# DeepRec-AI/DeepRec

Measured on AMD Instinct MI355X. Metric: samples/sec (whole node) DLRM Criteo-TB-shaped synthetic, higher is better.
Workload: dtype bf16; 1 GPU; model=dlrm, global_batch=8192, seq_len=1, parallelism=single, hip_graph=True, optimizer=adamasync, embedding_dim=16, num_tables=26

## Files before the change

### deeprec_amd/ops/hip/dense_kernels.hip

```cpp

#include "hip_common.h"

#include <algorithm>

namespace py = pybind11;

namespace {

using bf16 = __hip_bfloat16;
using bf16x8 = __attribute__((ext_vector_type(8))) short;
using f32x4 = __attribute__((ext_vector_type(4))) float;

__device__ __forceinline__ short act_grad_u16(short g, short o, int act) {
  const float ov = bf2f_u16(o);
  if (act == 1) return ov > 0.0f ? g : (short)0;
  return f2bf_u16(bf2f_u16(g) * ov * (1.0f - ov));
}

__device__ __forceinline__ bf16x8 load_frag_row(const short* __restrict__ src,
                                                int r, int k0, int rows,
                                                int cols) {
  bf16x8 out;
  if (r < rows && k0 + 7 < cols) {
    const short* p = src + (int64_t)r * cols + k0;
    out = *reinterpret_cast<const bf16x8*>(p);
  } else {
#pragma unroll
    for (int i = 0; i < 8; ++i) {
      short v = 0;
      if (r < rows && k0 + i < cols) v = src[(int64_t)r * cols + k0 + i];
      out[i] = v;
    }
  }
  return out;
}

__device__ __forceinline__ bf16x8 load_frag_col(const short* __restrict__ src,
                                                int c, int k0, int rows,
                                                int cols) {
  bf16x8 out;
#pragma unroll
  for (int i = 0; i < 8; ++i) {
    short v = 0;
    int r = k0 + i;
    if (r < rows && c < cols) v = src[(int64_t)r * cols + c];
    out[i] = v;
  }
  return out;
}

using bf16x4 = __attribute__((ext_vector_type(4))) short;
constexpr int TRT_COLS = 64;

__device__ __forceinline__ int trt_off(int row, int col) {
  const int sw = ((row >> 1) & 1) | ((row >> 2) & 2);
  return row * TRT_COLS + ((((col >> 4) ^ sw) << 4) | (col & 15));
}

__device__ __forceinline__ int trt_lane_off(int lane, int cb) {
  return trt_off(8 * (lane >> 4) + ((lane >> 2) & 3), cb + 4 * (lane & 3));
}

__device__ __forceinline__ bf16x4 lds_read_tr16(const short* p) {
  return __builtin_amdgcn_ds_read_tr16_b64_v4i16(
      (__attribute__((address_space(3))) bf16x4*)p);
}

__device__ __forceinline__ bf16x8 trt_frag(const short* p) {
  const bf16x4 lo = lds_read_tr16(p);
  const bf16x4 hi = lds_read_tr16(p + 4 * TRT_COLS);
  return __builtin_shufflevector(lo, hi, 0, 1, 2, 3, 4, 5, 6, 7);
}

constexpr int TRT_STAGE_THREADS = 256;
static_assert(TRT_STAGE_THREADS / 8 == 32, "a slab is 32 rows of 8 segments");
struct TrtStager {
  int row, col, off;
  __device__ __forceinline__ explicit TrtStager(int tid)
      : row(tid >> 3), col((tid & 7) * 8), off(trt_off(row, col)) {}
  __device__ __forceinline__ bf16x8 load(const short* __restrict__ src,
                                         int row0, int slab, int col0,
                                         int rows, int cols) const {
    return load_frag_row(src, row0 + slab * 32 + row, col0 + col, rows, cols);
  }
  __device__ __forceinline__ void store(short* tile, int slab,
                                        bf16x8 v) const {
    *reinterpret_cast<bf16x8*>(&tile[slab * 32 * TRT_COLS + off]) = v;
  }
};


__device__ __forceinline__ short fwd_act_u16(float acc, float bv, int act) {
  float v = acc + bv;
  if (act == 1 && v < 0.0f) v = 0.0f;
  else if (act == 2) v = 1.0f / (1.0f + __expf(-v));
  return f2bf_u16(v);
}

__device__ __forceinline__ void dx_store_tile(
    const f32x4 (&acc)[4], int lane, int m0, int c0, int kt, int M, int K,
    short* __restrict__ dX, const short* __restrict__ prev_out,
    int prev_act) {
#pragma unroll
  for (int t = 0; t < 4; ++t) {
    if (t >= kt) break;
    const int ck = c0 + t * 16 + (lane & 15);
    if (ck >= K) continue;
#pragma unroll
    for (int i = 0; i < 4; ++i) {
      int cm = m0 + (lane >> 4) * 4 + i;
      if (cm >= M) continue;
      short v = f2bf_u16(acc[t][i]);
      if (prev_out)
        v = act_grad_u16(v, prev_out[(int64_t)cm * K + ck], prev_act);
      dX[(int64_t)cm * K + ck] = v;
    }
  }
}

template <int NT>
__device__ __forceinline__ void dw_flush(const f32x4 (&acc)[NT], int lane,
                                         int n0, int k0, int N, int K,
                                         float* __restrict__ dW) {
#pragma unroll
  for (int t = 0; t < NT; ++t) {
    const int ck = k0 + t * 16 + (lane & 15);
    if (ck >= K) continue;
#pragma unroll
    for (int i = 0; i < 4; ++i) {
      int cn = n0 + (lane >> 4) * 4 + i;
      if (cn >= N) continue;
      atomicAdd(&dW[(int64_t)cn * K + ck], acc[t][i]);
    }
  }
}

__device__ __forceinline__ float dbias_add_frag(float bsum, bf16x8 gfrag) {
#pragma unroll
  for (int i = 0; i < 8; ++i) bsum += bf2f_u16(gfrag[i]);
  return bsum;
}

__device__ __forceinline__ void dbias_reduce_add(float bsum, int lane, int n0,
                                                 int N,
                                                 float* __restrict__ dbias) {
  float v = bsum;
  for (int off = 16; off < 64; off += 16)
    v += __shfl(bsum, (lane & 15) + off);
  const int cn = n0 + (lane & 15);
  if (lane < 16 && cn < N) atomicAdd(&dbias[cn], v);
}

template <int MT>
__global__ void k_linear_fwd_t(const short* __restrict__ A,
                               const short* __restrict__ W,
                               const float* __restrict__ bias, int M, int N,
                               int K, int act, short* __restrict__ C) {
  const int lane = threadIdx.x & 63;
  const int wave = threadIdx.x >> 6;
  const int ntiles64 = (N + 63) / 64;
  const int m0 = (blockIdx.x / ntiles64) * 64 * MT + wave * 16 * MT;
  const int n0 = (blockIdx.x % ntiles64) * 64;
  if (m0 >= M) return;
  const int col_b = n0 + (lane & 15);
  const int kgrp = (lane >> 4) * 8;
  f32x4 acc[MT][4] = {};
  const int nt = min(4, (N - n0 + 15) / 16);
  for (int k0 = 0; k0 < K; k0 += 32) {
    bf16x8 a[MT];
#pragma unroll
    for (int r = 0; r < MT; ++r)
      a[r] = load_frag_row(A, m0 + r * 16 + (lane & 15), k0 + kgrp, M, K);
#pragma unroll
    for (int t = 0; t < 4; ++t) {
      if (t >= nt) break;
      bf16x8 b = load_frag_row(W, col_b + t * 16, k0 + kgrp, N, K);
#pragma unroll
      for (int r = 0; r < MT; ++r)
        acc[r][t] = __builtin_amdgcn_mfma_f32_16x16x32_bf16(a[r], b,
                                                            acc[r][t], 0, 0,
                                                            0);
    }
  }
  __shared__ short cstage[4][16][72];
  const bool full_tile =
      (MT == 1) && (n0 + 64 <= N) && (m0 + 16 <= M) && ((N & 7) == 0);
  if (full_tile) {
#pragma unroll
    for (int t = 0; t < 4; ++t) {
      const int cn = t * 16 + (lane & 15);
      const float bv = bias ? bias[n0 + cn] : 0.0f;
#pragma unroll
      for (int i = 0; i < 4; ++i) {
        cstage[wave][(lane >> 4) * 4 + i][cn] =
            fwd_act_u16(acc[0][t][i], bv, act);
      }
    }
    __builtin_amdgcn_s_waitcnt(0);
#pragma unroll
    for (int half = 0; half < 2; ++half) {
      const int row = half * 8 + (lane >> 3);
      const int c8 = (lane & 7) * 8;
      bf16x8 vreg;
#pragma unroll
      for (int j = 0; j < 8; ++j) vreg[j] = cstage[wave][row][c8 + j];
      *reinterpret_cast<bf16x8*>(
          C + (int64_t)(m0 + row) * N + n0 + c8) = vreg;
    }
    return;
  }
#pragma unroll
  for (int r = 0; r < MT; ++r) {
#pragma unroll
    for (int t = 0; t < 4; ++t) {
      if (t >= nt) break;
      const int cn = n0 + t * 16 + (lane & 15);
      if (cn >= N) continue;
      const float bv = bias ? bias[cn] : 0.0f;
#pragma unroll
      for (int i = 0; i < 4; ++i) {
        int cm = m0 + r * 16 + (lane >> 4) * 4 + i;
        if (cm >= M) continue;
        C[(int64_t)cm * N + cn] = fwd_act_u16(acc[r][t][i], bv, act);
      }
    }
  }
}

__global__ void k_linear_dx(const short* __restrict__ G,
                            const short* __restrict__ W, int M, int N, int K,
                            short* __restrict__ dX,
                            const short* __restrict__ prev_out,
                            int prev_act) {
  const int lane = threadIdx.x & 63;
  const int wave = threadIdx.x >> 6;
  const int ktiles64 = (K + 63) / 64;
  const int m0 = (blockIdx.x / ktiles64) * 64 + wave * 16;
  const int c0 = (blockIdx.x % ktiles64) * 64;
  if (m0 >= M) return;
  const int row_g = m0 + (lane & 15);
  const int col_w = c0 + (lane & 15);
  const int kgrp = (lane >> 4) * 8;
  f32x4 acc[4] = {{0.f, 0.f, 0.f, 0.f}, {0.f, 0.f, 0.f, 0.f},
                  {0.f, 0.f, 0.f, 0.f}, {0.f, 0.f, 0.f, 0.f}};
  const int kt = min(4, (K - c0 + 15) / 16);
  for (int n0 = 0; n0 < N; n0 += 32) {
    bf16x8 a = load_frag_row(G, row_g, n0 + kgrp, M, N);
#pragma unroll
    for (int t = 0; t < 4; ++t) {
      if (t >= kt) break;
      bf16x8 b = load_frag_col(W, col_w + t * 16, n0 + kgrp, N, K);
      acc[t] = __builtin_amdgcn_mfma_f32_16x16x32_bf16(a, b, acc[t], 0, 0,
                                                       0);
    }
  }
  dx_store_tile(acc, lane, m0, c0, kt, M, K, dX, prev_out, prev_act);
}

constexpr int DX_NSUP = 256;
constexpr int DX_STAGE_BATCH = 2;
__global__ void k_linear_dx_lds(const short* __restrict__ G,
                                const short* __restrict__ W, int M, int N,
                                int K, short* __restrict__ dX,
                                const short* __restrict__ prev_out,
                                int prev_act) {
  __shared__ __attribute__((aligned(16))) short wl[DX_NSUP * TRT_COLS];
  const int lane = threadIdx.x & 63;
  const int wave = __builtin_amdgcn_readfirstlane(threadIdx.x >> 6);
  const int ktiles64 = (K + 63) / 64;
  const int m0 = (blockIdx.x / ktiles64) * 128 + wave * 32;
  const int c0 = (blockIdx.x % ktiles64) * 64;
  const int row_g0 = m0 + (lane & 15);
  const int row_g1 = m0 + 16 + (lane & 15);
  const int kgrp = (lane >> 4) * 8;
  const int kt = min(4, (K - c0 + 15) / 16);
  const TrtStager stg(threadIdx.x);
  int b_off[4];
#pragma unroll
  for (int t = 0; t < 4; ++t) b_off[t] = trt_lane_off(lane, t * 16);
  f32x4 acc[2][4] = {};
  for (int ns = 0; ns < N; ns += DX_NSUP) {
    const int nlen = min(DX_NSUP, N - ns);
    __syncthreads();
    {
      const int nstg = (nlen + 31) & ~31;
      for (int it0 = 0; it0 * 32 < nstg; it0 += DX_STAGE_BATCH) {
        bf16x8 v[DX_STAGE_BATCH];
#pragma unroll
        for (int j = 0; j < DX_STAGE_BATCH; ++j)
          v[j] = stg.load(W, ns, it0 + j, c0, N, K);
#pragma unroll
        for (int j = 0; j < DX_STAGE_BATCH; ++j) stg.store(wl, it0 + j, v[j]);
      }
    }
    __syncthreads();
    if (m0 >= M) continue;
    for (int n0 = 0; n0 < nlen; n0 += 32) {
      bf16x8 a0 = load_frag_row(G, row_g0, ns + n0 + kgrp, M, N);
      bf16x8 a1 = load_frag_row(G, row_g1, ns + n0 + kgrp, M, N);
#pragma unroll
      for (int t = 0; t < 4; ++t) {
        if (t >= kt) break;
        bf16x8 b = trt_frag(&wl[n0 * TRT_COLS + b_off[t]]);
        acc[0][t] =
            __builtin_amdgcn_mfma_f32_16x16x32_bf16(a0, b, acc[0][t], 0, 0,
                                                    0);
        acc[1][t] =
            __builtin_amdgcn_mfma_f32_16x16x32_bf16(a1, b, acc[1][t], 0, 0,
                                                    0);
      }
    }
  }
  if (m0 >= M) return;
#pragma unroll
  for (int rg = 0; rg < 2; ++rg)
    dx_store_tile(acc[rg], lane, m0 + rg * 16, c0, kt, M, K, dX, prev_out,
                  prev_act);
}

__global__ void k_linear_dw_lds(const short* __restrict__ G,
                                const short* __restrict__ A, int M, int N,
                                int K, float* __restrict__ dW,
                                float* __restrict__ dbias) {
  constexpr int CH = 128;
  constexpr int KG = 64;
  constexpr int APAD = 8;
  __shared__ short a_l[CH][KG + APAD];
  __shared__ short g_l[CH][16 + APAD];

  const int lane = threadIdx.x & 63;
  const int wave = threadIdx.x >> 6;
  const int tid = threadIdx.x;
  const int kgroups = (K + KG - 1) / KG;
  const int tiles_n = (N + 15) / 16;
  const int tile_id = blockIdx.x % (tiles_n * kgroups);
  const int chunk = blockIdx.x / (tiles_n * kgroups);
  const int n0 = (tile_id / kgroups) * 16;
  const int k0 = (tile_id % kgroups) * KG;
  const int mbeg = chunk * CH;

  {
    const int r_in_iter = tid >> 3;
    const int seg = tid & 7;
    for (int it = 0; it < CH / 32; ++it) {
      int r = it * 32 + r_in_iter;
      int m = mbeg + r;
      bf16x8 v = load_frag_row(A, m, k0 + seg * 8, M, K);
      *reinterpret_cast<bf16x8*>(&a_l[r][seg * 8]) = v;
    }
    const int r_g = tid >> 1;
    const int seg_g = tid & 1;
    bf16x8 v = load_frag_row(G, mbeg + r_g, n0 + seg_g * 8, M, N);
    *reinterpret_cast<bf16x8*>(&g_l[r_g][seg_g * 8]) = v;
  }
  __syncthreads();

  const int kw = wave * 16;
  const int col_a = kw + (lane & 15);
  const int col_g = lane & 15;
  const int kgrp = (lane >> 4) * 8;
  f32x4 acc[1] = {};
  float bsum = 0.0f;
  const bool do_bias = (dbias != nullptr) && (k0 == 0) && (wave == 0);
#pragma unroll
  for (int ms = 0; ms < CH; ms += 32) {
    bf16x8 afrag, gfrag;
#pragma unroll
    for (int i = 0; i < 8; ++i) {
      int m = ms + kgrp + i;
      gfrag[i] = g_l[m][col_g];
      afrag[i] = a_l[m][col_a];
    }
    acc[0] = __builtin_amdgcn_mfma_f32_16x16x32_bf16(gfrag, afrag, acc[0], 0,
                                                     0, 0);
    if (do_bias) bsum = dbias_add_frag(bsum, gfrag);
  }
  dw_flush<1>(acc, lane, n0, k0 + kw, N, K, dW);
  if (do_bias) dbias_reduce_add(bsum, lane, n0, N, dbias);
}

__global__ void k_linear_dw_lds64t(const short* __restrict__ G,
                                   const short* __restrict__ A, int M, int N,
                                   int K, int cpb,
                                   float* __restrict__ dW,
                                   float* __restrict__ dbias) {
  constexpr int CH = 128;
  __shared__ __attribute__((aligned(16))) short a_s[CH * TRT_COLS];
  __shared__ __attribute__((aligned(16))) short g_s[CH * TRT_COLS];
  const int lane = threadIdx.x & 63;
  const int wave = threadIdx.x >> 6;
  const int kgroups = (K + 63) / 64;
  const int ngroups = (N + 63) / 64;
  const int tile_id = blockIdx.x % (ngroups * kgroups);
  const int chunk0 = (blockIdx.x / (ngroups * kgroups)) * cpb;
  const int n0 = (tile_id / kgroups) * 64;
  const int k0 = (tile_id % kgroups) * 64;
  const TrtStager stg(threadIdx.x);
  const int g_off = trt_lane_off(lane, wave * 16);
  int a_off[4];
#pragma unroll
  for (int t = 0; t < 4; ++t) a_off[t] = trt_lane_off(lane, t * 16);
  f32x4 acc[4] = {};
  float bsum = 0.0f;
  const bool do_bias = (dbias != nullptr) && (k0 == 0);
  for (int c = 0; c < cpb; ++c) {
    const int mbeg = (chunk0 + c) * CH;
    if (mbeg >= M) break;
    if (c > 0) __syncthreads();
    bf16x8 va[CH / 32], vg[CH / 32];
#pragma unroll
    for (int it = 0; it < CH / 32; ++it) {
      va[it] = stg.load(A, mbeg, it, k0, M, K);
      vg[it] = stg.load(G, mbeg, it, n0, M, N);
    }
#pragma unroll
    for (int it = 0; it < CH / 32; ++it) {
      stg.store(a_s, it, va[it]);
      stg.store(g_s, it, vg[it]);
    }
    __syncthreads();
#pragma unroll
    for (int ms = 0; ms < CH; ms += 32) {
      bf16x8 gfrag = trt_frag(&g_s[ms * TRT_COLS + g_off]);
      if (do_bias) bsum = dbias_add_frag(bsum, gfrag);
#pragma unroll
      for (int t = 0; t < 4; ++t) {
        bf16x8 afrag = trt_frag(&a_s[ms * TRT_COLS + a_off[t]]);
        acc[t] =
            __builtin_amdgcn_mfma_f32_16x16x32_bf16(gfrag, afrag, acc[t],
                                                    0, 0, 0);
      }
    }
  }
  dw_flush<4>(acc, lane, n0 + wave * 16, k0, N, K, dW);
  if (do_bias) dbias_reduce_add(bsum, lane, n0 + wave * 16, N, dbias);
}

__device__ __forceinline__ float wave_sum(float v) {
#pragma unroll
  for (int off = 32; off; off >>= 1) v += __shfl_down(v, off);
  return __shfl(v, 0);
}

__global__ void k_l2norm_fwd(const short* __restrict__ X, int M, int N,
                             float eps, short* __restrict__ Y,
                             float* __restrict__ inv_norms) {
  const int lane = threadIdx.x & 63;
  const int row = blockIdx.x * 4 + (threadIdx.x >> 6);
  if (row >= M) return;
  const short* x = X + (int64_t)row * N;
  float ss = 0.0f;
  for (int j = lane; j < N; j += 64) {
    float v = bf2f_u16(x[j]);
    ss += v * v;
  }
  float inv = rsqrtf(fmaxf(wave_sum(ss), eps));
  short* y = Y + (int64_t)row * N;
  for (int j = lane; j < N; j += 64)
    y[j] = f2bf_u16(bf2f_u16(x[j]) * inv);
  if (lane == 0) inv_norms[row] = inv;
}

__global__ void k_l2norm_bwd(const short* __restrict__ dY,
                             const short* __restrict__ Y,
                             const float* __restrict__ inv_norms, int M,
                             int N, short* __restrict__ dX) {
  const int lane = threadIdx.x & 63;
  const int row = blockIdx.x * 4 + (threadIdx.x >> 6);
  if (row >= M) return;
  const short* dy = dY + (int64_t)row * N;
  const short* y = Y + (int64_t)row * N;
  float dot = 0.0f;
  for (int j = lane; j < N; j += 64)
    dot += bf2f_u16(y[j]) * bf2f_u16(dy[j]);
  dot = wave_sum(dot);
  const float inv = inv_norms[row];
  short* dx = dX + (int64_t)row * N;
  for (int j = lane; j < N; j += 64)
    dx[j] = f2bf_u16((bf2f_u16(dy[j]) - bf2f_u16(y[j]) * dot) * inv);
}

__global__ void k_zero_f32d(float* __restrict__ p, int64_t n) {
  const int64_t to16 =
      (int64_t)((16 - (reinterpret_cast<uintptr_t>(p) & 15)) & 15) >> 2;
  const int64_t head = to16 < n ? to16 : n;
  const int64_t nbody = (n - head) & ~3LL;
  float* body = p + head;
  int64_t i = (blockIdx.x * (int64_t)blockDim.x + threadIdx.x) * 4;
  int64_t stride = gridDim.x * (int64_t)blockDim.x * 4;
  for (; i < nbody; i += stride)
    *reinterpret_cast<float4*>(body + i) = make_float4(0.f, 0.f, 0.f, 0.f);
  if (blockIdx.x == 0 && threadIdx.x == 0) {
    for (int64_t j = 0; j < head; ++j) p[j] = 0.0f;
    for (int64_t j = head + nbody; j < n; ++j) p[j] = 0.0f;
  }
}

__global__ void k_dense_adam(float* __restrict__ w,
                             const float* __restrict__ g,
                             float* __restrict__ m, float* __restrict__ v,
                             short* __restrict__ w16,
                             const float* __restrict__ powers, int64_t n,
                             float lr, float beta1, float beta2, float eps,
                             float gscale) {
  const float lr_t = lr * sqrtf(1.0f - powers[1]) / (1.0f - powers[0]);
  int64_t i = blockIdx.x * (int64_t)blockDim.x + threadIdx.x;
  int64_t stride = gridDim.x * (int64_t)blockDim.x;
  for (; i < n; i += stride) {
    float gi = g[i] * gscale;
    float mn = beta1 * m[i] + (1.0f - beta1) * gi;
    float vn = beta2 * v[i] + (1.0f - beta2) * gi * gi;
    m[i] = mn;
    v[i] = vn;
    float wn = w[i] - lr_t * mn / (sqrtf(vn) + eps);
    w[i] = wn;
    if (w16) w16[i] = f2bf_u16(wn);
  }
}

template <int N>
__global__ void k_resln_fwd(const short* __restrict__ x,
                            const short* __restrict__ a,
                            const float* __restrict__ gamma,
                            const float* __restrict__ beta, int64_t M,
                            float eps, short* __restrict__ y,
                            short* __restrict__ z,
                            float* __restrict__ stats) {
  float gm[N], bt[N];
#pragma unroll
  for (int j = 0; j < N; ++j) {
    gm[j] = gamma[j];
    bt[j] = beta[j];
  }
  int64_t r = blockIdx.x * (int64_t)blockDim.x + threadIdx.x;
  int64_t stride = gridDim.x * (int64_t)blockDim.x;
  for (; r < M; r += stride) {
    const short* xp = x + r * N;
    const short* ap = a + r * N;
    float zv[N];
    float mean = 0.0f;
#pragma unroll
    for (int j = 0; j < N; ++j) {
      zv[j] = bf2f_u16(xp[j]) + bf2f_u16(ap[j]);
      mean += zv[j];
    }
    mean /= N;
    float var = 0.0f;
#pragma unroll
    for (int j = 0; j < N; ++j) {
      float d = zv[j] - mean;
      var += d * d;
    }
    float rstd = rsqrtf(var / N + eps);
    short* yp = y + r * N;
    short* zp = z + r * N;
#pragma unroll
    for (int j = 0; j < N; ++j) {
      zp[j] = f2bf_u16(zv[j]);
      yp[j] = f2bf_u16((zv[j] - mean) * rstd * gm[j] + bt[j]);
    }
    stats[r * 2] = mean;
    stats[r * 2 + 1] = rstd;
  }
}

template <int N>
__global__ void k_resln_bwd(const short* __restrict__ dy,
                            const short* __restrict__ z,
                            const float* __restrict__ stats,
                            const float* __restrict__ gamma, int64_t M,
                            short* __restrict__ dz,
                            float* __restrict__ dgamma,
                            float* __restrict__ dbeta) {
  __shared__ float ldg[N];
  __shared__ float ldb[N];
  for (int j = threadIdx.x; j < N; j += blockDim.x) {
    ldg[j] = 0.0f;
    ldb[j] = 0.0f;
  }
  __syncthreads();
  float gm[N], pg[N], pb[N];
#pragma unroll
  for (int j = 0; j < N; ++j) {
    gm[j] = gamma[j];
    pg[j] = 0.0f;
    pb[j] = 0.0f;
  }
  int64_t r = blockIdx.x * (int64_t)blockDim.x + threadIdx.x;
  int64_t stride = gridDim.x * (int64_t)blockDim.x;
  for (; r < M; r += stride) {
    const short* dyp = dy + r * N;
    const short* zp = z + r * N;
    const float mean = stats[r * 2];
    const float rstd = stats[r * 2 + 1];
    float s1 = 0.0f, s2 = 0.0f;
    float xh[N], g[N];
#pragma unroll
    for (int j = 0; j < N; ++j) {
      xh[j] = (bf2f_u16(zp[j]) - mean) * rstd;
      g[j] = bf2f_u16(dyp[j]);
      float gg = g[j] * gm[j];
      s1 += gg;
      s2 += gg * xh[j];
      pg[j] += g[j] * xh[j];
      pb[j] += g[j];
    }
    s1 /= N;
    s2 /= N;
    short* dzp = dz + r * N;
#pragma unroll
    for (int j = 0; j < N; ++j)
      dzp[j] = f2bf_u16((g[j] * gm[j] - s1 - xh[j] * s2) * rstd);
  }
#pragma unroll
  for (int j = 0; j < N; ++j) {
    atomicAdd(&ldg[j], pg[j]);
    atomicAdd(&ldb[j], pb[j]);
  }
  __syncthreads();
  for (int j = threadIdx.x; j < N; j += blockDim.x) {
    atomicAdd(&dgamma[j], ldg[j]);
    atomicAdd(&dbeta[j], ldb[j]);
  }
}

__global__ void k_act_bwd(const short* __restrict__ dY,
                          const short* __restrict__ out, int64_t n, int act,
                          short* __restrict__ G) {
  int64_t i = (blockIdx.x * (int64_t)blockDim.x + threadIdx.x) * 8;
  int64_t stride = gridDim.x * (int64_t)blockDim.x * 8;
  for (; i + 7 < n; i += stride) {
    bf16x8 g = *reinterpret_cast<const bf16x8*>(dY + i);
    bf16x8 o = *reinterpret_cast<const bf16x8*>(out + i);
    bf16x8 r;
#pragma unroll
    for (int j = 0; j < 8; ++j) r[j] = act_grad_u16(g[j], o[j], act);
    *reinterpret_cast<bf16x8*>(G + i) = r;
  }
  if (blockIdx.x == 0 && threadIdx.x == 0) {
    for (int64_t j = n & ~7LL; j < n; ++j)
      G[j] = act_grad_u16(dY[j], out[j], act);
  }
}

__global__ void k_pad_cast_bf16(const float* __restrict__ x, int64_t M, int K,
                                int KP, short* __restrict__ y) {
  const int gpr = (KP + 7) / 8;
  const int64_t ngroups = M * gpr;
  int64_t gi = blockIdx.x * (int64_t)blockDim.x + threadIdx.x;
  const int64_t stride = gridDim.x * (int64_t)blockDim.x;
  for (; gi < ngroups; gi += stride) {
    const int64_t r = gi / gpr;
    const int c0 = (int)(gi % gpr) * 8;
    bf16x8 v;
#pragma unroll
    for (int j = 0; j < 8; ++j) {
      short b = 0;
      if (c0 + j < K) {
        const float f = x[r * K + c0 + j];
        b = f != f ? (short)0x7fc0 : f2bf_u16(f);
      }
      v[j] = b;
    }
    short* dst = y + r * KP + c0;
    if ((KP & 7) == 0) {
      *reinterpret_cast<bf16x8*>(dst) = v;
    } else {
#pragma unroll
      for (int j = 0; j < 8; ++j)
        if (c0 + j < KP) dst[j] = v[j];
    }
  }
}

__global__ void k_interact_fwd(const short* __restrict__ feats, int B, int F,
                               int D, int P, int P_pad,
                               short* __restrict__ out) {
  const int lane = threadIdx.x & 63;
  const int wave = threadIdx.x >> 6;
  const int b = blockIdx.x * 4 + wave;
  extern __shared__ short lds[];
  short* f = lds + wave * F * D;
  const bool active = b < B;
  if (active) {
    const short* src = feats + (int64_t)b * F * D;
    for (int t = lane; t * 8 < F * D; t += 64) {
      *reinterpret_cast<bf16x8*>(f + t * 8) =
          *reinterpret_cast<const bf16x8*>(src + t * 8);
    }
  }
  __syncthreads();
  if (!active) return;
  short* dst = reinterpret_cast<short*>(out) + (int64_t)b * P_pad;
  for (int p = lane; p < P_pad; p += 64) {
    if (p >= P) {
      dst[p] = 0;
      continue;
    }
    int i = 0, rem = p, row = F - 1;
    while (rem >= row) {
      rem -= row;
      --row;
      ++i;
    }
    int j = i + 1 + rem;
    float acc = 0.0f;
    const short* fi = f + i * D;
    const short* fj = f + j * D;
    for (int d = 0; d < D; ++d)
      acc += bf2f_u16(fi[d]) * bf2f_u16(fj[d]);
    dst[p] = f2bf_u16(acc);
  }
}

__global__ void k_interact_cat_fwd(const short* __restrict__ bot,
                                   const short* __restrict__ emb, int B,
                                   int Fe, int D, int P, int P_pad,
                                   short* __restrict__ out) {
  const int lane = threadIdx.x & 63;
  const int wave = threadIdx.x >> 6;
  const int b = blockIdx.x * 4 + wave;
  const int F = Fe + 1;
  extern __shared__ short lds[];
  short* f = lds + wave * F * D;
  const bool active = b < B;
  if (active) {
    const short* bsrc = bot + (int64_t)b * D;
    for (int t = lane; t * 8 < D; t += 64)
      *reinterpret_cast<bf16x8*>(f + t * 8) =
          *reinterpret_cast<const bf16x8*>(bsrc + t * 8);
    const short* esrc = emb + (int64_t)b * Fe * D;
    for (int t = lane; t * 8 < Fe * D; t += 64)
      *reinterpret_cast<bf16x8*>(f + D + t * 8) =
          *reinterpret_cast<const bf16x8*>(esrc + t * 8);
  }
  __syncthreads();
  if (!active) return;
  short* dst = reinterpret_cast<short*>(out) + (int64_t)b * (D + P_pad);
  for (int d = lane; d < D; d += 64) dst[d] = f[d];
  dst += D;
  for (int p = lane; p < P_pad; p += 64) {
    if (p >= P) {
      dst[p] = 0;
      continue;
    }
    int i = 0, rem = p, row = F - 1;
    while (rem >= row) {
      rem -= row;
      --row;
      ++i;
    }
    int j = i + 1 + rem;
    float acc = 0.0f;
    const short* fi = f + i * D;
    const short* fj = f + j * D;
    for (int d = 0; d < D; ++d)
      acc += bf2f_u16(fi[d]) * bf2f_u16(fj[d]);
    dst[p] = f2bf_u16(acc);
  }
}

__global__ void k_interact_cat_bwd(const short* __restrict__ grad,
                                   const short* __restrict__ bot,
                                   const short* __restrict__ emb, int B,
                                   int Fe, int D, int P, int P_pad,
                                   short* __restrict__ dbot,
                                   short* __restrict__ demb) {
  const int lane = threadIdx.x & 63;
  const int wave = threadIdx.x >> 6;
  const int b = blockIdx.x * 4 + wave;
  const int F = Fe + 1;
  extern __shared__ short lds[];
  short* f = lds + wave * (F * D + ((P + 7) & ~7));
  short* g = f + F * D;
  const bool active = b < B;
  if (active) {
    const short* bsrc = bot + (int64_t)b * D;
    for (int t = lane; t * 8 < D; t += 64)
      *reinterpret_cast<bf16x8*>(f + t * 8) =
          *reinterpret_cast<const bf16x8*>(bsrc + t * 8);
    const short* esrc = emb + (int64_t)b * Fe * D;
    for (int t = lane; t * 8 < Fe * D; t += 64)
      *reinterpret_cast<bf16x8*>(f + D + t * 8) =
          *reinterpret_cast<const bf16x8*>(esrc + t * 8);
    const short* gsrc = grad + (int64_t)b * (D + P_pad) + D;
    for (int t = lane; t < P; t += 64) g[t] = gsrc[t];
  }
  __shared__ short plut[40 * 40];
  for (int t = threadIdx.x; t < F * F; t += blockDim.x) {
    int i = t / F, j = t % F;
    int lo = i < j ? i : j, hi = i < j ? j : i;
    plut[t] = (short)(i == j ? -1
                             : lo * F - (lo * (lo + 1)) / 2 + (hi - lo - 1));
  }
  __syncthreads();
  if (!active) return;
  const short* gdirect = grad + (int64_t)b * (D + P_pad);
  short* db = dbot + (int64_t)b * D;
  short* de = demb + (int64_t)b * Fe * D;
  for (int t = lane; t < F * D; t += 64) {
    int i = t / D, d = t % D;
    float acc = 0.0f;
    const short* prow = &plut[i * F];
    const short* fd = f + d;
#pragma unroll 4
    for (int j = 0; j < F; ++j) {
      int p = prow[j];
      if (p < 0) continue;
      acc += bf2f_u16(g[p]) * bf2f_u16(fd[j * D]);
    }
    if (i == 0) {
      db[d] = f2bf_u16(acc + bf2f_u16(gdirect[d]));
    } else {
      de[(i - 1) * D + d] = f2bf_u16(acc);
    }
  }
}

__global__ void k_interact_bwd(const short* __restrict__ grad,
                               const short* __restrict__ feats, int B, int F,
                               int D, int P, int P_pad,
                               short* __restrict__ dfeats) {
  const int lane = threadIdx.x & 63;
  const int wave = threadIdx.x >> 6;
  const int b = blockIdx.x * 4 + wave;
  extern __shared__ short lds[];
  short* f = lds + wave * (F * D + ((P + 7) & ~7));
  short* g = f + F * D;
  const bool active = b < B;
  if (active) {
    const short* fsrc = feats + (int64_t)b * F * D;
    const short* gsrc = grad + (int64_t)b * P_pad;
    for (int t = lane; t * 8 < F * D; t += 64)
      *reinterpret_cast<bf16x8*>(f + t * 8) =
          *reinterpret_cast<const bf16x8*>(fsrc + t * 8);
    for (int t = lane; t < P; t += 64) g[t] = gsrc[t];
  }
  __shared__ short plut[40 * 40];
  for (int t = threadIdx.x; t < F * F; t += blockDim.x) {
    int i = t / F, j = t % F;
    int lo = i < j ? i : j, hi = i < j ? j : i;
    plut[t] = (short)(i == j ? -1
                             : lo * F - (lo * (lo + 1)) / 2 + (hi - lo - 1));
  }
  __syncthreads();
  if (!active) return;
  short* dst = reinterpret_cast<short*>(dfeats) + (int64_t)b * F * D;
  for (int t = lane; t < F * D; t += 64) {
    int i = t / D, d = t % D;
    float acc = 0.0f;
    const short* prow = &plut[i * F];
    const short* fd = f + d;
#pragma unroll 4
    for (int j = 0; j < F; ++j) {
      int p = prow[j];
      if (p < 0) continue;
      acc += bf2f_u16(g[p]) * bf2f_u16(fd[j * D]);
    }
    dst[t] = f2bf_u16(acc);
  }
}

}


static const short* bf_ptr(const torch::Tensor& t) {
  return reinterpret_cast<const short*>(t.data_ptr<at::BFloat16>());
}
static short* bf_ptr_mut(torch::Tensor& t) {
  return reinterpret_cast<short*>(t.data_ptr<at::BFloat16>());
}

static void check_bf16_matrix(const torch::Tensor& t, const char* op,
                              const char* name) {
  TORCH_CHECK(t.is_cuda(), op, ": ", name, " must be on the GPU");
  TORCH_CHECK(t.dim() == 2, op, ": ", name, " must be 2-D, got ", t.dim(),
              "-D");
  TORCH_CHECK(t.scalar_type() == torch::kBFloat16, op, ": ", name,
              " must be bfloat16, got ", t.scalar_type());
  TORCH_CHECK(t.is_contiguous(), op, ": ", name,
              " must be contiguous (row-major)");
}

torch::Tensor linear_fwd(torch::Tensor x, torch::Tensor w_bf16,
                         torch::Tensor bias, int64_t act,
                         int64_t variant) {
  check_bf16_matrix(x, "linear_fwd", "x");
  check_bf16_matrix(w_bf16, "linear_fwd", "w");
  TORCH_CHECK(x.size(1) == w_bf16.size(1), "linear_fwd: x is [M,",
              x.size(1), "] but w is [N,", w_bf16.size(1), "]");
  int M = x.size(0), K = x.size(1), N = w_bf16.size(0);
  TORCH_CHECK(!bias.defined() || bias.numel() == 0 ||
                  (bias.numel() == N && bias.is_contiguous()),
              "linear_fwd: bias must be empty or contiguous [N]");
  TORCH_CHECK(variant >= -1 && variant <= 1, "linear_fwd: variant must be "
              "-1 (automatic), 0 (MT=1) or 1 (MT=2), got ", variant);
  auto out = torch::empty({M, N}, x.options());
  int tiles_n = (N + 63) / 64;
  const float* bp =
      bias.defined() && bias.numel() ? bias.data_ptr<float>() : nullptr;
  if (variant == 1) {
    int blocks = ((M + 127) / 128) * tiles_n;
    k_linear_fwd_t<2><<<blocks, 256, 0, current_hip_stream()>>>(
        bf_ptr(x), bf_ptr(w_bf16), bp, M, N, K, (int)act, bf_ptr_mut(out));
  } else {
    int blocks = ((M + 63) / 64) * tiles_n;
    k_linear_fwd_t<1><<<blocks, 256, 0, current_hip_stream()>>>(
        bf_ptr(x), bf_ptr(w_bf16), bp, M, N, K, (int)act, bf_ptr_mut(out));
  }
  return out;
}

torch::Tensor linear_dx(torch::Tensor g, torch::Tensor w_bf16,
                        c10::optional<torch::Tensor> prev_out,
                        int64_t prev_act) {
  check_bf16_matrix(g, "linear_dx", "g");
  check_bf16_matrix(w_bf16, "linear_dx", "w");
  TORCH_CHECK(g.size(1) == w_bf16.size(0), "linear_dx: g is [M,", g.size(1),
              "] but w is [", w_bf16.size(0), ",K]");
  int M = g.size(0), N = g.size(1), K = w_bf16.size(1);
  TORCH_CHECK(prev_act >= 0 && prev_act <= 2, "linear_dx: prev_act must be "
              "0 (none), 1 (relu) or 2 (sigmoid), got ", prev_act);
  const short* pp = nullptr;
  if (prev_out.has_value()) {
    check_bf16_matrix(*prev_out, "linear_dx", "prev_out");
    TORCH_CHECK(prev_out->size(0) == M && prev_out->size(1) == K,
                "linear_dx: prev_out is [", prev_out->size(0), ",",
                prev_out->size(1), "] but dX is [", M, ",", K, "]");
    if (prev_act != 0) pp = bf_ptr(*prev_out);
  } else {
    TORCH_CHECK(prev_act == 0, "linear_dx: prev_act without prev_out");
  }
  auto dx = torch::empty({M, K}, g.options());
  int tiles_k = (K + 63) / 64;
  if (N >= 128) {
    int blocks = ((M + 127) / 128) * tiles_k;
    k_linear_dx_lds<<<blocks, TRT_STAGE_THREADS, 0, current_hip_stream()>>>(
        bf_ptr(g), bf_ptr(w_bf16), M, N, K, bf_ptr_mut(dx), pp,
        (int)prev_act);
  } else {
    int blocks = ((M + 63) / 64) * tiles_k;
    k_linear_dx<<<blocks, 256, 0, current_hip_stream()>>>(
        bf_ptr(g), bf_ptr(w_bf16), M, N, K, bf_ptr_mut(dx), pp,
        (int)prev_act);
  }
  return dx;
}

static void zero_f32_launch(float* p, int64_t n) {
  k_zero_f32d<<<(int)std::clamp<int64_t>((n / 4 + 255) / 256, 1, 1024), 256,
                0, current_hip_stream()>>>(p, n);
}

static std::tuple<torch::Tensor, torch::Tensor> linear_dw_impl(
    const char* op, torch::Tensor g, torch::Tensor x, torch::Tensor ws,
    bool want_bias, int64_t variant, bool zero) {
  check_bf16_matrix(g, op, "g");
  check_bf16_matrix(x, op, "x");
  TORCH_CHECK(g.size(0) == x.size(0), op, ": g has ", g.size(0),
              " rows but x has ", x.size(0));
  TORCH_CHECK(variant == -1 || variant == 0 || variant == 2, op,
              ": variant must be -1 (automatic), 0 (k_linear_dw_lds) or 2 "
              "(k_linear_dw_lds64t), got ", variant);
  int M = g.size(0), N = g.size(1), K = x.size(1);
  int64_t ws_len = (int64_t)N * K + (want_bias ? N : 0);
  if (ws.defined()) {
    TORCH_CHECK(ws.is_cuda() && ws.is_contiguous() &&
                    ws.scalar_type() == torch::kFloat32 &&
                    ws.numel() == ws_len,
                op, ": ws must be a contiguous fp32 GPU tensor of ", ws_len,
                " elements");
  } else {
    ws = torch::empty({ws_len}, g.options().dtype(torch::kFloat32));
  }
  if (zero) zero_f32_launch(ws.data_ptr<float>(), ws_len);
  auto dw = ws.narrow(0, 0, (int64_t)N * K).view({N, K});
  auto db = want_bias ? ws.narrow(0, (int64_t)N * K, N) : torch::Tensor();
  int m_chunks = (M + 127) / 128;
  float* dbp = want_bias ? db.data_ptr<float>() : nullptr;
  if (variant < 0) variant = N >= 64 ? 2 : 0;
  if (variant == 2) {
    int tiles = ((N + 63) / 64) * ((K + 63) / 64);
    int cpb = std::max(1, (int)((int64_t)m_chunks * tiles / 512));
    int blocks = tiles * ((m_chunks + cpb - 1) / cpb);
    k_linear_dw_lds64t<<<blocks, TRT_STAGE_THREADS, 0,
                         current_hip_stream()>>>(
        bf_ptr(g), bf_ptr(x), M, N, K, cpb, dw.data_ptr<float>(), dbp);
  } else {
    int tiles = ((N + 15) / 16) * ((K + 63) / 64);
    k_linear_dw_lds<<<tiles * m_chunks, 256, 0, current_hip_stream()>>>(
        bf_ptr(g), bf_ptr(x), M, N, K, dw.data_ptr<float>(), dbp);
  }
  return {dw, db};
}

std::tuple<torch::Tensor, torch::Tensor> linear_dw(torch::Tensor g,
                                                   torch::Tensor x,
                                                   bool want_bias,
                                                   int64_t variant) {
  return linear_dw_impl("linear_dw", g, x, torch::Tensor(), want_bias,
                        variant, true);
}

std::tuple<torch::Tensor, torch::Tensor> linear_dw_out(torch::Tensor g,
                                                       torch::Tensor x,
                                                       torch::Tensor ws,
                                                       bool want_bias,
                                                       int64_t variant,
                                                       bool zero) {
  TORCH_CHECK(ws.defined(), "linear_dw_out: ws is undefined");
  return linear_dw_impl("linear_dw_out", g, x, ws, want_bias, variant, zero);
}

void zero_f32(torch::Tensor ws) {
  TORCH_CHECK(ws.is_cuda() && ws.dim() == 1 && ws.is_contiguous() &&
                  ws.scalar_type() == torch::kFloat32,
              "zero_f32: ws must be a contiguous 1-D fp32 GPU tensor");
  if (ws.numel() == 0) return;
  zero_f32_launch(ws.data_ptr<float>(), ws.numel());
}

torch::Tensor pad_cast_bf16(torch::Tensor x, int64_t k_pad) {
  TORCH_CHECK(x.is_cuda() && x.dim() == 2 && x.is_contiguous() &&
                  x.scalar_type() == torch::kFloat32,
              "pad_cast_bf16: x must be a contiguous 2-D fp32 GPU tensor");
  int64_t M = x.size(0), K = x.size(1);
  TORCH_CHECK(k_pad >= K, "pad_cast_bf16: k_pad ", k_pad, " < K ", K);
  TORCH_CHECK(k_pad < (1 << 30), "pad_cast_bf16: k_pad ", k_pad,
              " is out of range (< 2^30)");
  auto y = torch::empty({M, k_pad}, x.options().dtype(torch::kBFloat16));
  if (M == 0 || k_pad == 0) return y;
  int64_t groups = M * ((k_pad + 7) / 8);
  int blocks = (int)std::clamp<int64_t>((groups + 255) / 256, 1, 4096);
  k_pad_cast_bf16<<<blocks, 256, 0, current_hip_stream()>>>(
      x.data_ptr<float>(), M, (int)K, (int)k_pad, bf_ptr_mut(y));
  return y;
}

std::tuple<torch::Tensor, torch::Tensor, torch::Tensor> resln_fwd(
    torch::Tensor x, torch::Tensor a, torch::Tensor gamma,
    torch::Tensor beta, double eps) {
  TORCH_CHECK(x.scalar_type() == torch::kBFloat16 && x.is_contiguous());
  int64_t M = x.numel() / x.size(-1);
  int N = x.size(-1);
  TORCH_CHECK(N <= 64, "resln: row width must be <= 64");
  auto y = torch::empty_like(x);
  auto z = torch::empty_like(x);
  auto stats = torch::empty({M, 2}, x.options().dtype(torch::kFloat32));
  if (M == 0) return {y, z, stats};
  TORCH_CHECK(N == 16 || N == 32 || N == 64, "resln: N must be 16/32/64");
  int blocks = (int)std::min<int64_t>((M + 255) / 256, 4096);
#define RESLN_FWD(NV) \
  k_resln_fwd<NV><<<blocks, 256, 0, current_hip_stream()>>>( \
      bf_ptr(x), bf_ptr(a), gamma.data_ptr<float>(), \
      beta.data_ptr<float>(), M, (float)eps, bf_ptr_mut(y), \
      bf_ptr_mut(z), stats.data_ptr<float>())
  if (N == 16) RESLN_FWD(16);
  else if (N == 32) RESLN_FWD(32);
  else RESLN_FWD(64);
#undef RESLN_FWD
  return {y, z, stats};
}

std::tuple<torch::Tensor, torch::Tensor, torch::Tensor> resln_bwd(
    torch::Tensor dy, torch::Tensor z, torch::Tensor stats,
    torch::Tensor gamma) {
  int64_t M = z.numel() / z.size(-1);
  int N = z.size(-1);
  auto dz = torch::empty_like(z);
  auto opts = gamma.options();
  auto dgamma = torch::empty({N}, opts);
  auto dbeta = torch::empty({N}, opts);
  auto stream = current_hip_stream();
  k_zero_f32d<<<1, 64, 0, stream>>>(dgamma.data_ptr<float>(), N);
  k_zero_f32d<<<1, 64, 0, stream>>>(dbeta.data_ptr<float>(), N);
  if (M == 0) return {dz, dgamma, dbeta};
  auto dyc = dy.contiguous();
  int blocks = (int)std::min<int64_t>((M + 256 * 8 - 1) / (256 * 8), 4096);
  blocks = std::max(blocks, 64);
#define RESLN_BWD(NV) \
  k_resln_bwd<NV><<<blocks, 256, 0, stream>>>( \
      bf_ptr(dyc), bf_ptr(z), stats.data_ptr<float>(), \
      gamma.data_ptr<float>(), M, bf_ptr_mut(dz), \
      dgamma.data_ptr<float>(), dbeta.data_ptr<float>())
  if (N == 16) RESLN_BWD(16);
  else if (N == 32) RESLN_BWD(32);
  else RESLN_BWD(64);
#undef RESLN_BWD
  return {dz, dgamma, dbeta};
}

void dense_adam(torch::Tensor w, torch::Tensor g, torch::Tensor m,
                torch::Tensor v, torch::Tensor w16, torch::Tensor powers,
                double lr, double beta1, double beta2, double eps,
                double gscale) {
  int64_t n = w.numel();
  if (n == 0) return;
  short* w16p = (w16.defined() && w16.numel())
                    ? reinterpret_cast<short*>(w16.data_ptr<at::BFloat16>())
                    : nullptr;
  int blocks = (int)std::min<int64_t>((n + 255) / 256, 4096);
  k_dense_adam<<<blocks, 256, 0, current_hip_stream()>>>(
      w.data_ptr<float>(), g.data_ptr<float>(), m.data_ptr<float>(),
      v.data_ptr<float>(), w16p, powers.data_ptr<float>(), n, (float)lr,
      (float)beta1, (float)beta2, (float)eps, (float)gscale);
}

torch::Tensor act_bwd(torch::Tensor dy, torch::Tensor out, int64_t act) {
  auto g = torch::empty_like(dy);
  int64_t n = dy.numel();
  int blocks = (int)std::min<int64_t>((n / 8 + 255) / 256, 4096);
  k_act_bwd<<<std::max(blocks, 1), 256, 0, current_hip_stream()>>>(
      bf_ptr(dy), bf_ptr(out), n, (int)act, bf_ptr_mut(g));
  return g;
}

torch::Tensor interact_fwd(torch::Tensor feats, int64_t p_pad) {
  TORCH_CHECK(feats.scalar_type() == torch::kBFloat16 &&
              feats.is_contiguous());
  int B = feats.size(0), F = feats.size(1), D = feats.size(2);
  int P = F * (F - 1) / 2;
  TORCH_CHECK((F * D) % 8 == 0, "F*D must be a multiple of 8");
  auto out = torch::empty({B, p_pad}, feats.options());
  int blocks = (B + 3) / 4;
  size_t lds = 4 * (size_t)F * D * sizeof(short);
  k_interact_fwd<<<blocks, 256, lds, current_hip_stream()>>>(
      bf_ptr(feats), B, F, D, P, (int)p_pad, bf_ptr_mut(out));
  return out;
}

torch::Tensor interact_bwd(torch::Tensor grad, torch::Tensor feats) {
  int B = feats.size(0), F = feats.size(1), D = feats.size(2);
  TORCH_CHECK(F <= 40, "interact_bwd: pair LUT supports F <= 40");
  int P = F * (F - 1) / 2;
  int P_pad = grad.size(1);
  auto dfeats = torch::empty_like(feats);
  int blocks = (B + 3) / 4;
  size_t lds = 4 * (size_t)(F * D + ((P + 7) & ~7)) * sizeof(short);
  k_interact_bwd<<<blocks, 256, lds, current_hip_stream()>>>(
      bf_ptr(grad.contiguous()), bf_ptr(feats), B, F, D, P, P_pad,
      bf_ptr_mut(dfeats));
  return dfeats;
}

torch::Tensor interact_cat_fwd(torch::Tensor bot, torch::Tensor emb,
                               int64_t p_pad) {
  TORCH_CHECK(bot.scalar_type() == torch::kBFloat16 && bot.is_contiguous());
  TORCH_CHECK(emb.scalar_type() == torch::kBFloat16 && emb.is_contiguous());
  int B = emb.size(0), Fe = emb.size(1), D = emb.size(2);
  int F = Fe + 1;
  int P = F * (F - 1) / 2;
  TORCH_CHECK(D % 8 == 0, "D must be a multiple of 8");
  auto out = torch::empty({B, D + p_pad}, emb.options());
  int blocks = (B + 3) / 4;
  size_t lds = 4 * (size_t)F * D * sizeof(short);
  k_interact_cat_fwd<<<blocks, 256, lds, current_hip_stream()>>>(
      bf_ptr(bot), bf_ptr(emb), B, Fe, D, P, (int)p_pad, bf_ptr_mut(out));
  return out;
}

std::tuple<torch::Tensor, torch::Tensor> interact_cat_bwd(
    torch::Tensor grad, torch::Tensor bot, torch::Tensor emb) {
  int B = emb.size(0), Fe = emb.size(1), D = emb.size(2);
  int F = Fe + 1;
  TORCH_CHECK(F <= 40, "interact: pair LUT supports F <= 40");
  int P = F * (F - 1) / 2;
  int P_pad = grad.size(1) - D;
  auto dbot = torch::empty_like(bot);
  auto demb = torch::empty_like(emb);
  int blocks = (B + 3) / 4;
  size_t lds = 4 * (size_t)(F * D + ((P + 7) & ~7)) * sizeof(short);
  k_interact_cat_bwd<<<blocks, 256, lds, current_hip_stream()>>>(
      bf_ptr(grad.contiguous()), bf_ptr(bot), bf_ptr(emb), B, Fe, D, P,
      P_pad, bf_ptr_mut(dbot), bf_ptr_mut(demb));
  return {dbot, demb};
}

std::tuple<torch::Tensor, torch::Tensor> l2norm_fwd(torch::Tensor x,
                                                    double eps) {
  TORCH_CHECK(x.scalar_type() == torch::kBFloat16 && x.is_contiguous());
  int M = x.size(0), N = x.size(1);
  auto y = torch::empty_like(x);
  auto inv = torch::empty({M}, x.options().dtype(torch::kFloat32));
  k_l2norm_fwd<<<(M + 3) / 4, 256, 0, current_hip_stream()>>>(
      bf_ptr(x), M, N, (float)eps, bf_ptr_mut(y), inv.data_ptr<float>());
  return {y, inv};
}

torch::Tensor l2norm_bwd(torch::Tensor dy, torch::Tensor y,
                         torch::Tensor inv) {
  int M = y.size(0), N = y.size(1);
  auto dx = torch::empty_like(y);
  k_l2norm_bwd<<<(M + 3) / 4, 256, 0, current_hip_stream()>>>(
      bf_ptr(dy.contiguous()), bf_ptr(y), inv.data_ptr<float>(), M, N,
      bf_ptr_mut(dx));
  return dx;
}

void register_dense(py::module_& mod) {
  mod.def("l2norm_fwd", &l2norm_fwd);
  mod.def("l2norm_bwd", &l2norm_bwd);
  mod.def("interact_fwd", &interact_fwd);
  mod.def("interact_bwd", &interact_bwd);
  mod.def("interact_cat_fwd", &interact_cat_fwd);
  mod.def("interact_cat_bwd", &interact_cat_bwd);
  mod.def("linear_fwd", &linear_fwd, py::arg("x"), py::arg("w"),
          py::arg("bias"), py::arg("act"), py::arg("variant") = -1);
  mod.def("linear_dx", &linear_dx, py::arg("g"), py::arg("w"),
          py::arg("prev_out") = py::none(), py::arg("prev_act") = 0);
  mod.def("linear_dw", &linear_dw, py::arg("g"), py::arg("x"),
          py::arg("want_bias"), py::arg("variant") = -1);
  mod.def("linear_dw_out", &linear_dw_out, py::arg("g"), py::arg("x"),
          py::arg("ws"), py::arg("want_bias"), py::arg("variant") = -1,
          py::arg("zero") = true);
  mod.def("zero_f32", &zero_f32, py::arg("ws"));
  mod.def("pad_cast_bf16", &pad_cast_bf16, py::arg("x"), py::arg("k_pad"));
  mod.def("dense_adam", &dense_adam);
  mod.def("resln_fwd", &resln_fwd);
  mod.def("resln_bwd", &resln_bwd);
  mod.def("act_bwd", &act_bwd);
}
```

Baseline: 15.01 million samples/sec.

## Double-buffer operand loads in linear forward kernel with edge/interior specialization

Rewrites the MFMA main loop of the forward linear kernel to prefetch the next K-step's A and W fragments into a second register buffer while the current step's MFMAs run. Interior tiles get a template path without bounds checks, and edge tiles clamp row pointers and zero-fill instead of doing per-element guarded loads. A K tail path handles non-multiple-of-32 K, and __launch_bounds__(256) is added. The goal is to hide global load latency and cut branch overhead, at the cost of higher register pressure and more code.

Measured after the change: 15.58 million samples/sec (median of 6 runs). 3.8% higher.

```diff
diff --git a/deeprec_amd/ops/hip/dense_kernels.hip b/deeprec_amd/ops/hip/dense_kernels.hip
--- a/deeprec_amd/ops/hip/dense_kernels.hip
+++ b/deeprec_amd/ops/hip/dense_kernels.hip
@@ -152,7 +152,102 @@
 }
 
 template <int MT>
-__global__ void k_linear_fwd_t(const short* __restrict__ A,
+struct FwdStep {
+  bf16x8 a[MT];
+  bf16x8 b[4];
+};
+
+typedef bf16x8 bf16x8_u __attribute__((aligned(2)));
+
+template <int MT, bool EDGE>
+__device__ __forceinline__ void fwd_accumulate(const short* __restrict__ A,
+                                               const short* __restrict__ W,
+                                               int M, int N, int K, int m0,
+                                               int n0, int lane,
+                                               f32x4 (&acc)[MT][4]) {
+  const int kgrp = (lane >> 4) * 8;
+  const short* ap[MT];
+  const short* bp[4];
+  bool a_ok[MT], b_ok[4];
+#pragma unroll
+  for (int r = 0; r < MT; ++r) {
+    const int row = m0 + r * 16 + (lane & 15);
+    a_ok[r] = !EDGE || row < M;
+    ap[r] = A + (int64_t)(EDGE ? min(row, M - 1) : row) * K + kgrp;
+  }
+#pragma unroll
+  for (int t = 0; t < 4; ++t) {
+    const int row = n0 + t * 16 + (lane & 15);
+    b_ok[t] = !EDGE || row < N;
+    bp[t] = W + (int64_t)(EDGE ? min(row, N - 1) : row) * K + kgrp;
+  }
+  auto load = [&](FwdStep<MT>& s, int koff) {
+#pragma unroll
+    for (int r = 0; r < MT; ++r)
+      s.a[r] = *reinterpret_cast<const bf16x8_u*>(ap[r] + koff);
+#pragma unroll
+    for (int t = 0; t < 4; ++t)
+      s.b[t] = *reinterpret_cast<const bf16x8_u*>(bp[t] + koff);
+    __builtin_amdgcn_sched_barrier(0);
+  };
+  auto zero_fill = [&](FwdStep<MT>& s, bool kin) {
+    const bf16x8 zero = {};
+#pragma unroll
+    for (int r = 0; r < MT; ++r) s.a[r] = (a_ok[r] && kin) ? s.a[r] : zero;
+#pragma unroll
+    for (int t = 0; t < 4; ++t) s.b[t] = (b_ok[t] && kin) ? s.b[t] : zero;
+  };
+  auto mfma = [&](const FwdStep<MT>& s) {
+#pragma unroll
+    for (int t = 0; t < 4; ++t)
+#pragma unroll
+      for (int r = 0; r < MT; ++r)
+        acc[r][t] = __builtin_amdgcn_mfma_f32_16x16x32_bf16(
+            s.a[r], s.b[t], acc[r][t], 0, 0, 0);
+  };
+  auto step = [&](FwdStep<MT>& s) {
+    if (EDGE) zero_fill(s, true);
+    mfma(s);
+  };
+
+  const int nfull = K / 32;
+  FwdStep<MT> s0, s1;
+  if (nfull > 0) {
+    load(s0, 0);
+    int i = 0;
+    for (; i + 2 < nfull; i += 2) {
+      load(s1, (i + 1) * 32);
+      step(s0);
+      load(s0, (i + 2) * 32);
+      step(s1);
+    }
+    if (i + 2 == nfull) {
+      load(s1, (i + 1) * 32);
+      step(s0);
+      step(s1);
+    } else {
+      step(s0);
+    }
+  }
+  const int kt = nfull * 32;
+  if (kt == K) return;
+  if ((K & 7) == 0) {
+    const bool kin = kt + kgrp < K;
+    load(s0, kin ? kt : -kgrp);
+    zero_fill(s0, kin);
+  } else {
+#pragma unroll
+    for (int r = 0; r < MT; ++r)
+      s0.a[r] = load_frag_row(A, m0 + r * 16 + (lane & 15), kt + kgrp, M, K);
+#pragma unroll
+    for (int t = 0; t < 4; ++t)
+      s0.b[t] = load_frag_row(W, n0 + t * 16 + (lane & 15), kt + kgrp, N, K);
+  }
+  mfma(s0);
+}
+
+template <int MT>
+__global__ void __launch_bounds__(256) k_linear_fwd_t(const short* __restrict__ A,
                                const short* __restrict__ W,
                                const float* __restrict__ bias, int M, int N,
                                int K, int act, short* __restrict__ C) {
@@ -162,26 +257,12 @@
   const int m0 = (blockIdx.x / ntiles64) * 64 * MT + wave * 16 * MT;
   const int n0 = (blockIdx.x % ntiles64) * 64;
   if (m0 >= M) return;
-  const int col_b = n0 + (lane & 15);
-  const int kgrp = (lane >> 4) * 8;
   f32x4 acc[MT][4] = {};
   const int nt = min(4, (N - n0 + 15) / 16);
-  for (int k0 = 0; k0 < K; k0 += 32) {
-    bf16x8 a[MT];
-#pragma unroll
-    for (int r = 0; r < MT; ++r)
-      a[r] = load_frag_row(A, m0 + r * 16 + (lane & 15), k0 + kgrp, M, K);
-#pragma unroll
-    for (int t = 0; t < 4; ++t) {
-      if (t >= nt) break;
-      bf16x8 b = load_frag_row(W, col_b + t * 16, k0 + kgrp, N, K);
-#pragma unroll
-      for (int r = 0; r < MT; ++r)
-        acc[r][t] = __builtin_amdgcn_mfma_f32_16x16x32_bf16(a[r], b,
-                                                            acc[r][t], 0, 0,
-                                                            0);
-    }
-  }
+  if (m0 + 16 * MT <= M && n0 + 64 <= N)
+    fwd_accumulate<MT, false>(A, W, M, N, K, m0, n0, lane, acc);
+  else
+    fwd_accumulate<MT, true>(A, W, M, N, K, m0, n0, lane, acc);
   __shared__ short cstage[4][16][72];
   const bool full_tile =
       (MT == 1) && (n0 + 64 <= N) && (m0 + 16 <= M) && ((N & 7) == 0);
```
